# nogu-atsu/ENARF-GAN

Measured on AMD Instinct MI355X. Metric: rendered rays/sec (128^2, 64 samples/ray, 24 bones), higher is better.
Workload: dtype f32 (MLP products as 3-term split fp16 on MFMA, fp32 accumulate)

## Files before the change

enarf-gan_amd/csrc/enarf_tasks.h:

```cpp
#pragma once
#include "enarf_march.h"

namespace enarf {

constexpr unsigned ST_NONE = 0, ST_COARSE = 1, ST_FINE = 2;
__device__ __forceinline__ unsigned pack_ctl(unsigned gen, unsigned stage, unsigned tiles, unsigned next) {
    return (gen << 18) | (stage << 16) | (tiles << 8) | next;
}
__device__ __forceinline__ unsigned ctl_next(unsigned c) { return c & 0xFFu; }
__device__ __forceinline__ unsigned ctl_tiles(unsigned c) { return (c >> 8) & 0xFFu; }
__device__ __forceinline__ unsigned ctl_stage(unsigned c) { return (c >> 16) & 3u; }
__device__ __forceinline__ unsigned ctl_gen(unsigned c) { return c >> 18; }

constexpr int SH_QCUR = 0;
constexpr int SH_DEAD = 1;
constexpr int SH_INFLIGHT = 2;
constexpr int SH_PENDING = 3;
constexpr int SH_CTXB = 4;
constexpr int SH_SWITCHING = 5;
constexpr int SH_ERROR = 6;
constexpr int SH_FIRST = 7;
constexpr int SH_QCOUNTS = 8;
constexpr int SH_BTAB = SH_QCOUNTS + kQueues * kClasses;
constexpr int SH_PENDFLAG = SH_BTAB + 132;
constexpr int kSharedWords = SH_PENDFLAG + 16;
constexpr int kMaxSlots = 16;
constexpr unsigned kIdleLimit = 1u << 21;

template <int MODE>
__host__ __device__ inline int tasks_lds_floats(int P, int slots) {
    return lds_mlp_floats<MODE>() + 144 + P * kLdsPartStride + P * kLdsCanonStride + slots * kSlotWords + kSharedWords;
}

__device__ __forceinline__ unsigned wave_lds_add(unsigned *p, unsigned v, int lane) {
    unsigned r = 0;
    if (lane == 0) r = atomicAdd(p, v);
    return (unsigned)__builtin_amdgcn_readfirstlane((int)r);
}
__device__ __forceinline__ unsigned wave_lds_cas(unsigned *p, unsigned expect, unsigned desired, int lane) {
    unsigned r = 0;
    if (lane == 0) r = atomicCAS(p, expect, desired);
    return (unsigned)__builtin_amdgcn_readfirstlane((int)r);
}
__device__ __forceinline__ void lds_release() { __builtin_amdgcn_fence(__ATOMIC_RELEASE, "workgroup", "local"); }
__device__ __forceinline__ void lds_acquire() { __builtin_amdgcn_fence(__ATOMIC_ACQUIRE, "workgroup", "local"); }

struct TaskQueue {
    unsigned int *heads;
    const uint32_t *lists;
    const RayRec *recs;
    unsigned *sh;
    long long band;
    int home;
    __device__ __forceinline__ void init(void *workspace, int epoch, int B, int n, unsigned *shared, int tid) {
        unsigned int *wsh = reinterpret_cast<unsigned int *>(reinterpret_cast<char *>(workspace) + ws_header_off(epoch));
        heads = wsh + kWsHeadsOff;
        recs = reinterpret_cast<const RayRec *>(reinterpret_cast<const char *>(workspace) + ws_records_off());
        lists = reinterpret_cast<const uint32_t *>(reinterpret_cast<const char *>(workspace) + ws_list_off((long long)B * n));
        sh = shared;
        band = ws_band_size(B, n);
        home = xcc_id() & (kQueues - 1);
        if (tid < kQueues * kClasses) sh[SH_QCOUNTS + tid] = wsh[kWsCountsOff + tid];
    }
    __device__ __forceinline__ int pop(RayRec &rec, int lane) {
        int rid = -1;
        if (lane == 0) {
            unsigned cur = sh[SH_QCUR];
            int cls = (int)(cur >> 4), tries = (int)(cur & 15u);
            int lid = -1, idx = 0;
            while (cls < kClasses) {
                while (tries < kQueues) {
                    const int q = (home + tries) & (kQueues - 1);
                    const int l = q * kClasses + cls;
                    const unsigned len = sh[SH_QCOUNTS + l];
                    if (len != 0) {
                        const unsigned j = atomicAdd(heads + l * kWsHeadStride, 1u);
                        if (j < len) { lid = l; idx = (int)j; break; }
                    }
                    tries += 1;
                }
                if (lid >= 0) break;
                cls += 1;
                tries = 0;
            }
            atomicMax(&sh[SH_QCUR], (unsigned)(cls * 16 + tries));
            if (lid >= 0) rid = (int)lists[(size_t)lid * (size_t)band + (size_t)idx];
        }
        rid = __builtin_amdgcn_readfirstlane(rid);
        if (rid >= 0) rec = recs[rid];
        return rid;
    }
};

}

namespace enarf {

typedef const __attribute__((address_space(4))) enarf_render_args *RenderArgsK;
__device__ __forceinline__ RenderArgsK kernel_render_args() {
    return (RenderArgsK)__builtin_amdgcn_kernarg_segment_ptr();
}
__device__ __forceinline__ const enarf_render_args &render_args_ref(RenderArgsK a) { return *(const enarf_render_args *)a; }

struct MarchCtx {
    unsigned *slots;
    unsigned *sh;
    const float *btab;
    int nslots, nct, nft;
};

struct MarchCounters { unsigned pairs, tiles, rays, rounds, skipped; };

template <int SPL>
__device__ __forceinline__ void draw_sorted_uniforms(const enarf_render_args &a, uint32_t rid, int Nf, int lane, float usort[SPL]) {
    float esum[SPL];
    uint32_t r1_first = 0;
#pragma unroll
    for (int s = 0; s < SPL; ++s) {
        uint32_t rnd[4];
        philox4x32((uint32_t)(a.ray_id_base + rid), (uint32_t)((a.ray_id_base + rid) >> 32), (uint32_t)(64 * s + lane), 0x454E4152u, (uint32_t)a.seed, (uint32_t)(a.seed >> 32), rnd);
        esum[s] = (64 * s + lane < Nf) ? -__logf(1.0f - u32_to_unit(rnd[0])) : 0.0f;
        if (s == 0) r1_first = rnd[1];
    }
    wv_scan_incl<SPL>(esum, lane);
    const float etot = __shfl(esum[SPL - 1], 63) - __logf(1.0f - u32_to_unit((uint32_t)__shfl((int)r1_first, 0)));
#pragma unroll
    for (int s = 0; s < SPL; ++s) usort[s] = fminf(esum[s] / etot, 0.99999994f);
}

template <int SPL>
__device__ __forceinline__ void bins_from_cdf(int Nc, int Nf, const float cdf[SPL], const float usort[SPL], int lane, float bin[SPL]) {
    const float total = wv_get<SPL>(cdf, Nc - 1);
#pragma unroll
    for (int s = 0; s < SPL; ++s) {
        const float target = usort[s] * total;
        int lo = 0, hi = Nc - 1;
#pragma unroll
        for (int it = 0; it < 5 + SPL; ++it) {
            const int mid = (lo + hi) >> 1;
            const float c = wv_get<SPL>(cdf, mid);
            if (lo < hi) { if (c > target) hi = mid; else lo = mid + 1; }
        }
        const float c_hi = wv_get<SPL>(cdf, lo), c_lo = wv_get<SPL>(cdf, max(lo - 1, 0));
        const float below = (lo > 0) ? c_lo : 0.0f;
        const float frac = fminf(fmaxf((target - below) / (c_hi - below), 0.0f), 0.99999994f);
        bin[s] = (64 * s + lane < Nf) ? ((float)lo + frac) / (float)Nc : 3.0e38f;
    }
}

template <int SPL>
__device__ __forceinline__ void ray_sample_stage(const enarf_render_args &a, const float *l_btab, unsigned *sw, uint32_t rid,
                                                 float dmin, float dmax, const float usort[SPL], int mult_w, int lane) {
    const int P = a.P, Nc = a.Nc, Nf = a.Nf, n = a.n;
    const int b = (int)(rid / (uint32_t)n), ray = (int)(rid - (uint32_t)b * (uint32_t)n);
    const float *l_ch = reinterpret_cast<const float *>(sw + SL_CH), *l_cwmax = reinterpret_cast<const float *>(sw + SL_CWMAX);
    const uint32_t *l_cbits = sw + SL_CBITS;
    float *l_bins = reinterpret_cast<float *>(sw + SL_BINS);
    int *l_skip = reinterpret_cast<int *>(sw + SL_SKIP);
    float bin[SPL];
    float dd[SPL], cs[SPL], T[SPL], wgt[SPL], ws[SPL], wl[SPL], wr[SPL];
#pragma unroll
    for (int s = 0; s < SPL; ++s) {
        const int e = 64 * s + lane;
        const bool active = e < Nc;
        const int ci = min(e, Nc - 1);
        const float den = active ? density_head(l_ch[ci], l_cbits[ci], l_cwmax[ci], mult_w, P) : 0.0f;
        if (a.dbg_coarse_density && active) a.dbg_coarse_density[((size_t)b * n + ray) * Nc + e] = den;
        const float b0 = l_btab[ci], b1 = l_btab[ci + 1];
        const float delta = exact_lerp(dmin, dmax, b1) - exact_lerp(dmin, dmax, b0);
        dd[s] = active ? den * delta * a.render_scale : 0.0f;
        cs[s] = dd[s];
    }
    wv_scan_incl<SPL>(cs, lane);
#pragma unroll
    for (int s = 0; s < SPL; ++s) {
        T[s] = expf(-(cs[s] - dd[s]));
        wgt[s] = (64 * s + lane < Nc) ? T[s] * (1.0f - expf(-dd[s])) : 0.0f;
    }
    wv_prev<SPL>(wgt, wl, lane);
    wv_next<SPL>(wgt, wr, lane);
#pragma unroll
    for (int s = 0; s < SPL; ++s) {
        const int e = 64 * s + lane;
        if (e >= Nc - 1) wr[s] = 0.0f;
        ws[s] = (e < Nc) ? (fmaxf(wl[s], wgt[s]) + fmaxf(wgt[s], wr[s])) / 2.0f + 0.01f : 0.0f;
    }
    if (a.bins) {
#pragma unroll
        for (int s = 0; s < SPL; ++s) bin[s] = a.bins[((size_t)b * n + ray) * Nf + min(64 * s + lane, Nf - 1)];
    } else {
        float cdf[SPL];
#pragma unroll
        for (int s = 0; s < SPL; ++s) cdf[s] = ws[s];
        wv_scan_incl<SPL>(cdf, lane);
        bins_from_cdf<SPL>(Nc, Nf, cdf, usort, lane, bin);
    }
#pragma unroll
    for (int s = 0; s < SPL; ++s) {
        l_bins[64 * s + lane] = bin[s];
        if (a.dbg_bins && 64 * s + lane < Nf) a.dbg_bins[((size_t)b * n + ray) * Nf + 64 * s + lane] = bin[s];
    }
#pragma unroll
    for (int t = 0; t < 4 * SPL; ++t) {
        bool skip = false;
        if (a.early_stop_eps > 0.0f) {
            const float b_first = wv_get<SPL>(bin, min(16 * t, Nf - 1));
            const int jbin = min(max((int)(b_first * (float)Nc), 0), Nc - 1);
            skip = wv_get<SPL>(T, jbin) < a.early_stop_eps;
        }
        if (lane == 0) l_skip[t] = skip ? 1 : 0;
    }
}

template <int SPL>
__device__ __noinline__ void slot_sample_stage(RenderArgsK ak, const float *l_btab, unsigned *sw, int mult_w, int lane) {
    const enarf_render_args &a = render_args_ref(ak);
    const RayRec rec = *reinterpret_cast<const RayRec *>(sw + SL_REC);
    const uint32_t rid = sw[SL_RID];
    float usort[SPL] = {};
    if (!a.bins) draw_sorted_uniforms<SPL>(a, rid, a.Nf, lane, usort);
    ray_sample_stage<SPL>(a, l_btab, sw, rid, rec.dmin, rec.dmax, usort, mult_w, lane);
}

template <int SPL>
__device__ __forceinline__ void ray_composite_stage(const enarf_render_args &a, const unsigned *sw, uint32_t rid, float dmin,
                                                    float dmax, int mult_w, int lane) {
    const int P = a.P, Nf = a.Nf, n = a.n;
    const int b = (int)(rid / (uint32_t)n), ray = (int)(rid - (uint32_t)b * (uint32_t)n);
    const float *l_fh = reinterpret_cast<const float *>(sw + SL_FH), *l_fwmax = reinterpret_cast<const float *>(sw + SL_FWMAX);
    const float *l_bins = reinterpret_cast<const float *>(sw + SL_BINS);
    const uint32_t *l_fbits = sw + SL_FBITS;
    const bool dbgq = (a.dbg_fine_density != nullptr);
    float fdepth[SPL], dnext[SPL], den[SPL], cr[SPL], cg[SPL], cb[SPL], dd[SPL], cs[SPL];
#pragma unroll
    for (int s = 0; s < SPL; ++s) {
        const int e = 64 * s + lane;
        const int ci = min(e, Nf - 1);
        const bool have = e < (dbgq ? Nf : Nf - 1);
        const uint32_t bits = l_fbits[ci];
        den[s] = have ? density_head(l_fh[3 * kMaxSamples + ci], bits, l_fwmax[ci], mult_w, P) : 0.0f;
        cr[s] = tanhf(l_fh[ci]); cg[s] = tanhf(l_fh[kMaxSamples + ci]); cb[s] = tanhf(l_fh[2 * kMaxSamples + ci]);
        fdepth[s] = exact_lerp(dmin, dmax, l_bins[64 * s + lane]);
        if (dbgq && e < Nf) {
            const size_t o = ((size_t)b * n + ray) * Nf + e;
            a.dbg_fine_density[o] = den[s];
            if (a.dbg_fine_valid) a.dbg_fine_valid[o] = bits;
            if (a.dbg_fine_color) {
                a.dbg_fine_color[(((size_t)b * 3 + 0) * n + ray) * Nf + e] = cr[s];
                a.dbg_fine_color[(((size_t)b * 3 + 1) * n + ray) * Nf + e] = cg[s];
                a.dbg_fine_color[(((size_t)b * 3 + 2) * n + ray) * Nf + e] = cb[s];
            }
        }
    }
    wv_next<SPL>(fdepth, dnext, lane);
#pragma unroll
    for (int s = 0; s < SPL; ++s) {
        dd[s] = (64 * s + lane < Nf - 1) ? den[s] * (dnext[s] - fdepth[s]) * a.render_scale : 0.0f;
        cs[s] = dd[s];
    }
    wv_scan_incl<SPL>(cs, lane);
    float wgt[SPL], vr[SPL], vg[SPL], vb[SPL], vd[SPL];
#pragma unroll
    for (int s = 0; s < SPL; ++s) {
        const bool seg = 64 * s + lane < Nf - 1;
        const float T = expf(-(cs[s] - dd[s]));
        wgt[s] = seg ? T * (1.0f - expf(-dd[s])) : 0.0f;
        vr[s] = wgt[s] * cr[s]; vg[s] = wgt[s] * cg[s]; vb[s] = wgt[s] * cb[s];
        vd[s] = seg ? (wgt[s] * 1.0f) / fdepth[s] : 0.0f;
    }
    const float o_r = wv_sum<SPL>(vr), o_g = wv_sum<SPL>(vg), o_b = wv_sum<SPL>(vb);
    const float o_m = wv_sum<SPL>(wgt), o_d = wv_sum<SPL>(vd);
    if (lane == 0) {
        a.color[((size_t)b * 3 + 0) * n + ray] = o_r;
        a.color[((size_t)b * 3 + 1) * n + ray] = o_g;
        a.color[((size_t)b * 3 + 2) * n + ray] = o_b;
        a.mask[(size_t)b * n + ray] = o_m;
        a.disparity[(size_t)b * n + ray] = o_d;
    }
#pragma unroll
    for (int s = 0; s < SPL; ++s) {
        const int e = 64 * s + lane;
        if (a.fine_weights && e < Nf - 1) a.fine_weights[((size_t)b * n + ray) * (Nf - 1) + e] = wgt[s];
        if (a.fine_depth && e < Nf) a.fine_depth[((size_t)b * n + ray) * Nf + e] = fdepth[s];
    }
}

template <int SPL>
__device__ __noinline__ void slot_composite_stage(RenderArgsK ak, unsigned *sw, int mult_w, int lane) {
    const RayRec rec = *reinterpret_cast<const RayRec *>(sw + SL_REC);
    ray_composite_stage<SPL>(render_args_ref(ak), sw, sw[SL_RID], rec.dmin, rec.dmax, mult_w, lane);
}

struct RaySeg { float sx, sy, sz, ex, ey, ez; };
__device__ __forceinline__ RaySeg ray_segment(const RayRec &rec) {
    return {exact_mul(rec.dmin, rec.dx), exact_mul(rec.dmin, rec.dy), exact_mul(rec.dmin, rec.dz),
            exact_mul(rec.dmax, rec.dx), exact_mul(rec.dmax, rec.dy), exact_mul(rec.dmax, rec.dz)};
}

template <int MODE>
__device__ __forceinline__ void ray_tile(const enarf_render_args &a, const QueryCtx &S, const float *l_btab, const int *l_cand,
                                         int ncand, unsigned *sw, const RaySeg &g, bool fine, int t, int lane, MarchCounters &C) {
    const int Nc = a.Nc, Nf = a.Nf;
    const int j4 = lane >> 2, base = 16 * t, i = base + j4;
    const int N = fine ? Nf : Nc;
    const bool dbgq = (a.dbg_fine_density != nullptr);
    bool skip = false, active;
    float px, py, pz;
    if (!fine) {
        active = i < Nc;
        const int ci = min(i, Nc - 1);
        const float b0 = l_btab[ci], b1 = l_btab[ci + 1];
        px = exact_mid(exact_lerp(g.sx, g.ex, b1), exact_lerp(g.sx, g.ex, b0));
        py = exact_mid(exact_lerp(g.sy, g.ey, b1), exact_lerp(g.sy, g.ey, b0));
        pz = exact_mid(exact_lerp(g.sz, g.ez, b1), exact_lerp(g.sz, g.ez, b0));
    } else {
        skip = reinterpret_cast<const int *>(sw + SL_SKIP)[t] != 0;
        active = (i < (dbgq ? Nf : Nf - 1)) && !skip;
        const float bi = reinterpret_cast<const float *>(sw + SL_BINS)[min(i, Nf - 1)];
        px = exact_lerp(g.sx, g.ex, bi); py = exact_lerp(g.sy, g.ey, bi); pz = exact_lerp(g.sz, g.ez, bi);
    }
    const QueryDbg nodbg{nullptr, nullptr, 0, 0};
    f32x4 o;
    bool ran;
    uint32_t bits;
    float wmax;
    query_tile<MODE, false>(S, l_cand, ncand, px, py, pz, active, lane, o, ran, bits, wmax, nodbg, C.pairs, C.tiles, &C.rounds);
    float *heads = reinterpret_cast<float *>(sw + (fine ? SL_FH : SL_CH));
    if (lane < 16 && base + lane < N) {
        const int io = base + lane;
        if (fine) { heads[io] = o[0]; heads[kMaxSamples + io] = o[1]; heads[2 * kMaxSamples + io] = o[2]; heads[3 * kMaxSamples + io] = o[3]; }
        else heads[io] = o[3];
    }
    if (i < N && (lane & 3) == 0) {
        sw[(fine ? SL_FBITS : SL_CBITS) + i] = active ? bits : 0u;
        reinterpret_cast<float *>(sw + (fine ? SL_FWMAX : SL_CWMAX))[i] = wmax;
    }
    if (skip) C.skipped += 1;
}

template <int MODE>
__device__ __forceinline__ void ray_tile_task(const enarf_render_args &a, const MarchCtx &M, QueryCtx &S, unsigned *sw, bool fine,
                                              int t, int lane, MarchCounters &C) {
    const RayRec rec = *reinterpret_cast<const RayRec *>(sw + SL_REC);
    const uint32_t rid = (uint32_t)__builtin_amdgcn_readfirstlane((int)sw[SL_RID]);
    const int b = (int)(rid / (uint32_t)a.n);
    S.feat = a.feat_cl + (size_t)b * a.feat_batch_stride;
    S.mask = a.mask_planes + (size_t)b * a.mask_batch_stride;
    ray_tile<MODE>(a, S, M.btab, reinterpret_cast<const int *>(sw + SL_CAND), (int)sw[SL_NCAND], sw, ray_segment(rec), fine, t,
                   lane, C);
}

template <int SPL>
__device__ __forceinline__ void missed_ray_short_cut(RenderArgsK a, uint32_t rid, const RayRec &rec, const float cdf[SPL], int lane) {
    const int Nc = a->Nc, Nf = a->Nf, n = a->n;
    const int b = (int)(rid / (uint32_t)n), ray = (int)(rid - (uint32_t)b * (uint32_t)n);
    float bin[SPL];
    if (a->bins) {
#pragma unroll
        for (int s = 0; s < SPL; ++s) bin[s] = a->bins[((size_t)b * n + ray) * Nf + min(64 * s + lane, Nf - 1)];
    } else {
        float usort[SPL];
        draw_sorted_uniforms<SPL>(render_args_ref(a), rid, Nf, lane, usort);
        bins_from_cdf<SPL>(Nc, Nf, cdf, usort, lane, bin);
    }
    if (lane < 3) a->color[((size_t)b * 3 + lane) * n + ray] = 0.0f;
    if (lane == 3) a->mask[(size_t)b * n + ray] = 0.0f;
    if (lane == 4) a->disparity[(size_t)b * n + ray] = 0.0f;
#pragma unroll
    for (int s = 0; s < SPL; ++s) {
        const int e = 64 * s + lane;
        if (a->dbg_bins && e < Nf) a->dbg_bins[((size_t)b * n + ray) * Nf + e] = bin[s];
        if (a->fine_weights && e < Nf - 1) a->fine_weights[((size_t)b * n + ray) * (Nf - 1) + e] = 0.0f;
        if (a->fine_depth && e < Nf) a->fine_depth[((size_t)b * n + ray) * Nf + e] = exact_lerp(rec.dmin, rec.dmax, bin[s]);
    }
}

constexpr int kMissedChunk = 32;
template <int SPL>
__device__ __forceinline__ unsigned march_missed_rays(RenderArgsK ak, const float *l_btab, unsigned *scratch, int mult_w, int lane) {
    const int B = ak->B, n = ak->n, Nc = ak->Nc;
    const char *ws = reinterpret_cast<const char *>(ak->workspace);
    unsigned int *wsh = reinterpret_cast<unsigned int *>(const_cast<char *>(ws) + ws_header_off(ak->ws_epoch));
    const uint32_t *lists = reinterpret_cast<const uint32_t *>(ws + ws_list_off((long long)B * n));
    const RayRec *recs = reinterpret_cast<const RayRec *>(ws + ws_records_off());
    if (wsh[2] == 0u) return 0u;
    const long long band = ws_band_size(B, n);
    const int home = xcc_id() & (kQueues - 1);
    const bool general = ak->dbg_fine_density || ak->dbg_coarse_density;
    float cdf[SPL];
#pragma unroll
    for (int s = 0; s < SPL; ++s) cdf[s] = (64 * s + lane < Nc) ? (0.0f + 0.0f) / 2.0f + 0.01f : 0.0f;
    wv_scan_incl<SPL>(cdf, lane);
    unsigned done = 0;
    bool zeroed = false;
    for (int t = 0; t < kQueues; ++t) {
        const int l = ws_missed_list((home + t) & (kQueues - 1));
        const unsigned len = wsh[kWsCountsOff + l];
        if (len == 0u) continue;
        while (true) {
            unsigned j0 = 0;
            if (lane == 0) j0 = atomicAdd(wsh + kWsHeadsOff + l * kWsHeadStride, (unsigned)kMissedChunk);
            j0 = (unsigned)__builtin_amdgcn_readfirstlane((int)j0);
            if (j0 >= len) break;
            const unsigned j1 = min(j0 + (unsigned)kMissedChunk, len);
            for (unsigned j = j0; j < j1; ++j) {
                const uint32_t rid = (uint32_t)__builtin_amdgcn_readfirstlane((int)lists[(size_t)l * (size_t)band + j]);
                if (general) {
                    if (!zeroed) {
                        for (int i = lane; i < kSlotWords; i += 64) scratch[i] = 0u;
                        zeroed = true;
                    }
                    if (lane == 0) {
                        scratch[SL_RID] = rid;
                        *reinterpret_cast<RayRec *>(scratch + SL_REC) = recs[rid];
                    }
                    slot_sample_stage<SPL>(ak, l_btab, scratch, mult_w, lane);
                    slot_composite_stage<SPL>(ak, scratch, mult_w, lane);
                } else {
                    missed_ray_short_cut<SPL>(ak, rid, recs[rid], cdf, lane);
                }
                done += 1;
            }
        }
    }
    return done;
}

struct ImageCtx {
    const enarf_render_args *a;
    float *lds;
};

template <int MODE>
__device__ __forceinline__ void stage_image(RenderArgsK a, float *lds, int b, int lane) {
    QueryCtx tmp;
    float *unused;
    stage_common<MODE>(lds, tmp, unused, reinterpret_cast<const char *>(a->mlp_pack) + (size_t)b * kPackBytes,
                       a->parts + (size_t)b * a->P * kPartStride, a->canonical_pose, a->P, lane, 64);
}

__device__ __forceinline__ void publish_ray(const MarchCtx &M, unsigned *sw, int lane) {
    const RayRec rec = *reinterpret_cast<const RayRec *>(sw + SL_REC);
    const int ncand = build_cand_list(reinterpret_cast<int *>(sw + SL_CAND), rec.cand, lane);
    if (lane == 0) { sw[SL_NCAND] = (unsigned)ncand; sw[SL_DONE] = 0u; }
    lds_release();
    if (lane == 0) {
        const unsigned gen = (ctl_gen(sw[SL_CTL]) + 1u) & 0x3FFFu;
        __hip_atomic_store(&sw[SL_CTL], pack_ctl(gen, ST_COARSE, (unsigned)M.nct, 0u), __ATOMIC_RELAXED, __HIP_MEMORY_SCOPE_WORKGROUP);
    }
}

template <int MODE>
__device__ __forceinline__ void drain_point(RenderArgsK a, const MarchCtx &M, float *lds, int lane) {
    volatile unsigned *vsh = M.sh;
    while (true) {
        if (vsh[SH_PENDING] == 0u) return;
        if (wave_lds_cas(&M.sh[SH_SWITCHING], 0u, 1u, lane) != 0u) return;
        lds_acquire();
        unsigned best = 0xFFFFFFFFu;
        for (int s = 0; s < M.nslots; ++s)
            if (vsh[SH_PENDFLAG + s]) best = min(best, (unsigned)M.slots[s * kSlotWords + SL_RID]);
        if (best != 0xFFFFFFFFu) {
            const int b = (int)(best / (uint32_t)a->n);
            if ((unsigned)b != vsh[SH_CTXB]) {
                stage_image<MODE>(a, lds, b, lane);
                if (lane == 0) M.sh[SH_CTXB] = (unsigned)b;
            }
            lds_release();
            for (int s = 0; s < M.nslots; ++s) {
                unsigned *sw = M.slots + s * kSlotWords;
                if (vsh[SH_PENDFLAG + s] && (int)(sw[SL_RID] / (uint32_t)a->n) == b) {
                    if (lane == 0) { M.sh[SH_PENDFLAG + s] = 0u; atomicAdd(&M.sh[SH_PENDING], 0xFFFFFFFFu); atomicAdd(&M.sh[SH_INFLIGHT], 1u); }
                    publish_ray(M, sw, lane);
                }
            }
        }
        lds_release();
        if (lane == 0) __hip_atomic_store(&M.sh[SH_SWITCHING], 0u, __ATOMIC_RELAXED, __HIP_MEMORY_SCOPE_WORKGROUP);
        lds_release();
        lds_acquire();
        if (!(vsh[SH_INFLIGHT] == 0u && vsh[SH_PENDING] != 0u)) return;
    }
}

template <int MODE>
__device__ __forceinline__ void release_token(RenderArgsK a, const MarchCtx &M, float *lds, int lane) {
    lds_release();
    const unsigned before = wave_lds_add(&M.sh[SH_INFLIGHT], 0xFFFFFFFFu, lane);
    if (before == 1u) drain_point<MODE>(a, M, lds, lane);
}

template <int MODE>
__device__ __noinline__ unsigned refill_slot(RenderArgsK a, const MarchCtx M, TaskQueue tq, float *lds, int s, int lane) {
    unsigned popped = 0u;
    unsigned *sw = M.slots + s * kSlotWords;
    RayRec rec;
    int rid;
    volatile unsigned *vst = sw + SL_NEXT_STATE;
    unsigned ahead = *vst;
    while (ahead == 3u && reinterpret_cast<volatile unsigned *>(M.sh)[SH_ERROR] == 0u) { __builtin_amdgcn_s_sleep(2); ahead = *vst; }
    if (ahead == 3u) ahead = 2u;
    if (ahead == 1u) {
        lds_acquire();
        rid = (int)sw[SL_NEXT_RID];
        rec = *reinterpret_cast<const RayRec *>(sw + SL_NEXT_REC);
        lds_release();
        if (lane == 0) __hip_atomic_store(sw + SL_NEXT_STATE, 0u, __ATOMIC_RELAXED, __HIP_MEMORY_SCOPE_WORKGROUP);
    } else if (ahead == 2u) {
        rid = -1;
    } else {
        rid = tq.pop(rec, lane);
        if (rid >= 0) popped = 1u;
    }
    if (rid < 0) {
        if (lane == 0) atomicAdd(&M.sh[SH_DEAD], 1u);
        release_token<MODE>(a, M, lds, lane);
        return popped;
    }
    if (lane == 0) { sw[SL_RID] = (unsigned)rid; *reinterpret_cast<RayRec *>(sw + SL_REC) = rec; }
    const unsigned b = (unsigned)rid / (uint32_t)a->n;
    volatile unsigned *vsh = M.sh;
    if (b == vsh[SH_CTXB]) {
        publish_ray(M, sw, lane);
    } else {
        if (lane == 0) { M.sh[SH_PENDFLAG + s] = 1u; atomicAdd(&M.sh[SH_PENDING], 1u); }
        release_token<MODE>(a, M, lds, lane);
    }
    return popped;
}

__device__ __noinline__ unsigned prefetch_next_ray(TaskQueue tq, unsigned *sw, int lane) {
    if (wave_lds_cas(sw + SL_NEXT_STATE, 0u, 3u, lane) != 0u) return 0u;
    RayRec rec;
    const int rid = tq.pop(rec, lane);
    if (lane == 0 && rid >= 0) { sw[SL_NEXT_RID] = (unsigned)rid; *reinterpret_cast<RayRec *>(sw + SL_NEXT_REC) = rec; }
    lds_release();
    if (lane == 0) __hip_atomic_store(sw + SL_NEXT_STATE, rid >= 0 ? 1u : 2u, __ATOMIC_RELAXED, __HIP_MEMORY_SCOPE_WORKGROUP);
    return rid >= 0 ? 1u : 0u;
}

template <int MODE, int SPL, int NW>
__global__ __launch_bounds__(NW * 64, NW / 4) void march_kernel(const enarf_render_args a, int nslots, unsigned int *status) {
    extern __shared__ __attribute__((aligned(16))) float lds[];
    const int tid = threadIdx.x, lane = tid & 63, wave = tid >> 6;
    const int P = a.P, Nc = a.Nc, Nf = a.Nf;
    QueryCtx S;
    float *after;
    {
        float *l_mlp = lds, *l_bias = l_mlp + lds_mlp_floats<MODE>(), *l_parts = l_bias + 144;
        float *l_canon = l_parts + P * kLdsPartStride;
        after = l_canon + P * kLdsCanonStride;
        S.mlp = l_mlp; S.mlp_h = reinterpret_cast<const short *>(l_mlp); S.bias = l_bias; S.parts = l_parts; S.canon = l_canon;
    }
    S.feat = a.feat_cl; S.mask = a.mask_planes;
    S.H = a.H; S.W = a.W; S.P = P; S.mult_w = a.multiply_density_with_weight ? (a.uniform_part_weight ? 2 : 1) : 0;
    S.clamp_mask = a.clamp_mask; S.uniform_w = a.uniform_part_weight ? 1.0f / (float)P : 0.0f;
    MarchCtx M;
    M.slots = reinterpret_cast<unsigned *>(after);
    M.sh = M.slots + nslots * kSlotWords;
    M.btab = reinterpret_cast<const float *>(M.sh + SH_BTAB);
    M.nslots = nslots; M.nct = (Nc + 15) / 16; M.nft = (Nf + 15) / 16;
    TaskQueue tq;
    tq.init(a.workspace, a.ws_epoch, a.B, a.n, M.sh, tid);
    if (tid == 0) {
        M.sh[SH_QCUR] = 0u; M.sh[SH_DEAD] = 0u; M.sh[SH_PENDING] = 0u; M.sh[SH_CTXB] = 0xFFFFFFFFu; M.sh[SH_SWITCHING] = 0u;
        M.sh[SH_ERROR] = 0u;
        M.sh[SH_INFLIGHT] = (unsigned)nslots;
    }
    if (tid <= Nc) reinterpret_cast<float *>(M.sh + SH_BTAB)[tid] = linspace_sym(0.0f, 1.0f, Nc + 1, tid);
    for (int s = tid; s < nslots; s += NW * 64) {
        M.slots[s * kSlotWords + SL_CTL] = pack_ctl(0u, ST_NONE, 0u, 0u);
        M.slots[s * kSlotWords + SL_DONE] = 0u;
        M.slots[s * kSlotWords + SL_NEXT_STATE] = 0u;
        M.sh[SH_PENDFLAG + s] = 0u;
    }
    __syncthreads();

    MarchCounters C{0u, 0u, 0u, 0u, 0u};
    const RenderArgsK ak = kernel_render_args();
    if (wave < lds_mlp_floats<MODE>() / kSlotWords)
        C.rays += march_missed_rays<SPL>(ak, M.btab, reinterpret_cast<unsigned *>(lds) + wave * kSlotWords, S.mult_w, lane);
    __syncthreads();
    if (wave == 0) {
        RayRec rec;
        const int rid = tq.pop(rec, lane);
        if (lane == 0) {
            M.sh[SH_FIRST] = (unsigned)rid;
            if (rid >= 0) { M.slots[SL_RID] = (unsigned)rid; *reinterpret_cast<RayRec *>(M.slots + SL_REC) = rec; }
        }
        if (rid >= 0) C.rays += 1;
    }
    __syncthreads();
    const int first = (int)M.sh[SH_FIRST];
    if (first < 0) {
        if (a.counters && lane == 0 && C.rays) atomicAdd(&a.counters[2], (unsigned long long)C.rays);
        return;
    }
    {
        const int b0 = (int)((unsigned)first / (uint32_t)a.n);
        QueryCtx tmp;
        float *unused;
        stage_common<MODE>(lds, tmp, unused, reinterpret_cast<const char *>(a.mlp_pack) + (size_t)b0 * kPackBytes,
                           a.parts + (size_t)b0 * P * kPartStride, a.canonical_pose, P, tid, NW * 64);
        if (tid == 0) M.sh[SH_CTXB] = (unsigned)b0;
    }
    __syncthreads();
    if (wave == 0) publish_ray(M, M.slots, lane);
    for (int s = wave; s < nslots; s += NW)
        if (s != 0) C.rays += refill_slot<MODE>(ak, M, tq, lds, s, lane);

    volatile unsigned *vsl = M.slots;
    volatile unsigned *vsh = M.sh;
    unsigned idle = 0u;
    for (;;) {
        const unsigned c = (lane < nslots) ? vsl[lane * kSlotWords + SL_CTL] : 0u;
        const bool can = ctl_next(c) < ctl_tiles(c);
        const uint64_t bf = __ballot(can && ctl_stage(c) == ST_FINE), bc = __ballot(can && ctl_stage(c) == ST_COARSE);
        const uint64_t set = bf ? bf : bc;
        if (set) {
            const int start = wave % nslots;
            const uint64_t hi = (set >> start) << start;
            const int s = hi ? __builtin_ctzll(hi) : __builtin_ctzll(set);
            const unsigned old = (unsigned)__builtin_amdgcn_readlane((int)c, s);
            unsigned *sw = M.slots + s * kSlotWords;
            if (wave_lds_cas(&sw[SL_CTL], old, old + 1u, lane) != old) continue;
            lds_acquire();
            const bool fine = ctl_stage(old) == ST_FINE;
            idle = 0u;
            ray_tile_task<MODE>(a, M, S, sw, fine, (int)ctl_next(old), lane, C);
            lds_release();
            const unsigned d = wave_lds_add(&sw[SL_DONE], 1u, lane);
            if (d + 1u == ctl_tiles(old)) {
                lds_acquire();
                if (!fine) {
                    __builtin_amdgcn_s_setprio(3);
                    slot_sample_stage<SPL>(ak, M.btab, sw, S.mult_w, lane);
                    __builtin_amdgcn_s_setprio(0);
                    if (lane == 0) sw[SL_DONE] = 0u;
                    lds_release();
                    if (lane == 0)
                        __hip_atomic_store(&sw[SL_CTL], pack_ctl(ctl_gen(old), ST_FINE, (unsigned)M.nft, 0u), __ATOMIC_RELAXED,
                                           __HIP_MEMORY_SCOPE_WORKGROUP);
                    __builtin_amdgcn_s_setprio(1);
                    C.rays += prefetch_next_ray(tq, sw, lane);
                    __builtin_amdgcn_s_setprio(0);
                } else {
                    __builtin_amdgcn_s_setprio(3);
                    slot_composite_stage<SPL>(ak, sw, S.mult_w, lane);
                    C.rays += refill_slot<MODE>(ak, M, tq, lds, s, lane);
                    __builtin_amdgcn_s_setprio(0);
                }
            }
            continue;
        }
        if (vsh[SH_DEAD] >= (unsigned)nslots || vsh[SH_ERROR] != 0u) break;
        if (++idle > kIdleLimit) {
            if (lane == 0) {
                M.sh[SH_ERROR] = 1u;
                if (status) __hip_atomic_fetch_or(status, ENARF_STATUS_MARCH_WATCHDOG, __ATOMIC_RELAXED, __HIP_MEMORY_SCOPE_SYSTEM);
                if (a.counters) atomicAdd(&a.counters[7], 1ull);
                reinterpret_cast<unsigned int *>(reinterpret_cast<char *>(a.workspace) + ws_header_off(a.ws_epoch))[0] = 0xDEADu;
            }
            break;
        }
        __builtin_amdgcn_s_sleep(4);
    }
    if (a.counters && lane == 0) {
        atomicAdd(&a.counters[0], (unsigned long long)C.pairs);
        atomicAdd(&a.counters[1], (unsigned long long)C.tiles);
        atomicAdd(&a.counters[2], (unsigned long long)C.rays);
        atomicAdd(&a.counters[3], (unsigned long long)C.rounds);
        atomicAdd(&a.counters[4], (unsigned long long)C.skipped);
    }
}

}
```

Before: 66.97 million.

## Replace slot-scan tile scheduler with LDS ring queues of tile tokens

Waves used to poll every slot's control word and claim tiles by CAS on the per-slot counter. Now publishing a stage pushes one token per tile into a fine or a coarse ring buffer in LDS, and waves pop tokens by CAS on the ring head, with generation tags to drop stale tokens. Idle waves back off with an escalating sleep instead of a fixed one. This is meant to cut polling and CAS contention on slot words, but it adds ring bookkeeping and LDS space and carries ordering risk.

```diff
diff --git a/enarf-gan_amd/csrc/enarf_ring.h b/enarf-gan_amd/csrc/enarf_ring.h
--- /dev/null
+++ b/enarf-gan_amd/csrc/enarf_ring.h
@@ -0,0 +1,38 @@
+#pragma once
+
+#if defined(__HIPCC__) || defined(__CUDACC__)
+#define ENARF_RING_FN __host__ __device__ inline
+#else
+#define ENARF_RING_FN inline
+#endif
+
+namespace enarf {
+
+constexpr int kMaxSlots = 16;
+constexpr int kRingMaxTiles = 8;
+constexpr int kRingLog2 = 7;
+constexpr int kRingSize = 1 << kRingLog2;
+static_assert(kRingSize == kMaxSlots * kRingMaxTiles, "a ring holds every slot's largest stage");
+
+constexpr int RQ_HEAD_FINE = 0, RQ_TAIL_FINE = 1, RQ_HEAD_COARSE = 2, RQ_TAIL_COARSE = 3;
+constexpr int RQ_FINE = 4, RQ_COARSE = RQ_FINE + kRingSize;
+constexpr int kRingWords = RQ_COARSE + kRingSize;
+constexpr unsigned kRingEmptyEntry = 0xFFFF0000u;
+
+ENARF_RING_FN unsigned ring_index(unsigned pos) { return pos & (unsigned)(kRingSize - 1); }
+ENARF_RING_FN unsigned ring_lap(unsigned pos) { return (pos >> kRingLog2) & 0xFFFFu; }
+ENARF_RING_FN unsigned ring_token(unsigned pos, unsigned gen, unsigned slot, unsigned tile) {
+    return (ring_lap(pos) << 16) | ((gen & 0xFFu) << 8) | ((slot & 15u) << 4) | (tile & 15u);
+}
+ENARF_RING_FN unsigned token_tile(unsigned t) { return t & 15u; }
+ENARF_RING_FN unsigned token_slot(unsigned t) { return (t >> 4) & 15u; }
+ENARF_RING_FN unsigned token_gen(unsigned t) { return (t >> 8) & 0xFFu; }
+ENARF_RING_FN bool ring_entry_ready(unsigned entry, unsigned pos) { return (entry >> 16) == ring_lap(pos); }
+ENARF_RING_FN bool token_is_current(unsigned t, unsigned gen) { return token_gen(t) == (gen & 0xFFu); }
+ENARF_RING_FN int ring_pick(unsigned head_fine, unsigned tail_fine, unsigned head_coarse, unsigned tail_coarse) {
+    if (head_fine != tail_fine) return 0;
+    if (head_coarse != tail_coarse) return 1;
+    return -1;
+}
+
+}
diff --git a/enarf-gan_amd/csrc/enarf_tasks.h b/enarf-gan_amd/csrc/enarf_tasks.h
--- a/enarf-gan_amd/csrc/enarf_tasks.h
+++ b/enarf-gan_amd/csrc/enarf_tasks.h
@@ -1,5 +1,6 @@
 #pragma once
 #include "enarf_march.h"
+#include "enarf_ring.h"
 
 namespace enarf {
 
@@ -23,13 +24,13 @@
 constexpr int SH_QCOUNTS = 8;
 constexpr int SH_BTAB = SH_QCOUNTS + kQueues * kClasses;
 constexpr int SH_PENDFLAG = SH_BTAB + 132;
-constexpr int kSharedWords = SH_PENDFLAG + 16;
-constexpr int kMaxSlots = 16;
+constexpr int kSharedWords = SH_PENDFLAG + kMaxSlots;
 constexpr unsigned kIdleLimit = 1u << 21;
 
 template <int MODE>
 __host__ __device__ inline int tasks_lds_floats(int P, int slots) {
-    return lds_mlp_floats<MODE>() + 144 + P * kLdsPartStride + P * kLdsCanonStride + slots * kSlotWords + kSharedWords;
+    return lds_mlp_floats<MODE>() + 144 + P * kLdsPartStride + P * kLdsCanonStride + slots * kSlotWords + kSharedWords +
+           kRingWords + 3;
 }
 
 __device__ __forceinline__ unsigned wave_lds_add(unsigned *p, unsigned v, int lane) {
@@ -44,6 +45,24 @@
 }
 __device__ __forceinline__ void lds_release() { __builtin_amdgcn_fence(__ATOMIC_RELEASE, "workgroup", "local"); }
 __device__ __forceinline__ void lds_acquire() { __builtin_amdgcn_fence(__ATOMIC_ACQUIRE, "workgroup", "local"); }
+
+__device__ __forceinline__ void ring_push(unsigned *rq, bool fine, unsigned slot, unsigned gen, int ntiles, int lane) {
+    lds_release();
+    const unsigned t0 = wave_lds_add(&rq[fine ? RQ_TAIL_FINE : RQ_TAIL_COARSE], (unsigned)ntiles, lane);
+    if (lane < ntiles) {
+        const unsigned pos = t0 + (unsigned)lane;
+        __hip_atomic_store(&rq[(fine ? RQ_FINE : RQ_COARSE) + ring_index(pos)], ring_token(pos, gen, slot, (unsigned)lane),
+                           __ATOMIC_RELAXED, __HIP_MEMORY_SCOPE_WORKGROUP);
+    }
+}
+__device__ __forceinline__ bool ring_take(unsigned *rq, bool fine, unsigned head, unsigned &token, int lane) {
+    const unsigned e = (unsigned)__builtin_amdgcn_readfirstlane(
+        (int)reinterpret_cast<volatile unsigned *>(rq)[(fine ? RQ_FINE : RQ_COARSE) + ring_index(head)]);
+    if (!ring_entry_ready(e, head)) return false;
+    if (wave_lds_cas(&rq[fine ? RQ_HEAD_FINE : RQ_HEAD_COARSE], head, head + 1u, lane) != head) return false;
+    token = e;
+    return true;
+}
 
 struct TaskQueue {
     unsigned int *heads;
@@ -105,6 +124,7 @@
 struct MarchCtx {
     unsigned *slots;
     unsigned *sh;
+    unsigned *rq;
     const float *btab;
     int nslots, nct, nft;
 };
@@ -439,15 +459,13 @@
                        a->parts + (size_t)b * a->P * kPartStride, a->canonical_pose, a->P, lane, 64);
 }
 
-__device__ __forceinline__ void publish_ray(const MarchCtx &M, unsigned *sw, int lane) {
+__device__ __forceinline__ void publish_ray(const MarchCtx &M, int s, int lane) {
+    unsigned *sw = M.slots + s * kSlotWords;
     const RayRec rec = *reinterpret_cast<const RayRec *>(sw + SL_REC);
     const int ncand = build_cand_list(reinterpret_cast<int *>(sw + SL_CAND), rec.cand, lane);
-    if (lane == 0) { sw[SL_NCAND] = (unsigned)ncand; sw[SL_DONE] = 0u; }
-    lds_release();
-    if (lane == 0) {
-        const unsigned gen = (ctl_gen(sw[SL_CTL]) + 1u) & 0x3FFFu;
-        __hip_atomic_store(&sw[SL_CTL], pack_ctl(gen, ST_COARSE, (unsigned)M.nct, 0u), __ATOMIC_RELAXED, __HIP_MEMORY_SCOPE_WORKGROUP);
-    }
+    const unsigned gen = (ctl_gen(reinterpret_cast<volatile unsigned *>(sw)[SL_CTL]) + 1u) & 0x3FFFu;
+    if (lane == 0) { sw[SL_NCAND] = (unsigned)ncand; sw[SL_DONE] = 0u; sw[SL_CTL] = pack_ctl(gen, ST_COARSE, (unsigned)M.nct, 0u); }
+    ring_push(M.rq, false, (unsigned)s, gen, M.nct, lane);
 }
 
 template <int MODE>
@@ -471,7 +489,7 @@
                 unsigned *sw = M.slots + s * kSlotWords;
                 if (vsh[SH_PENDFLAG + s] && (int)(sw[SL_RID] / (uint32_t)a->n) == b) {
                     if (lane == 0) { M.sh[SH_PENDFLAG + s] = 0u; atomicAdd(&M.sh[SH_PENDING], 0xFFFFFFFFu); atomicAdd(&M.sh[SH_INFLIGHT], 1u); }
-                    publish_ray(M, sw, lane);
+                    publish_ray(M, s, lane);
                 }
             }
         }
@@ -521,7 +539,7 @@
     const unsigned b = (unsigned)rid / (uint32_t)a->n;
     volatile unsigned *vsh = M.sh;
     if (b == vsh[SH_CTXB]) {
-        publish_ray(M, sw, lane);
+        publish_ray(M, s, lane);
     } else {
         if (lane == 0) { M.sh[SH_PENDFLAG + s] = 1u; atomicAdd(&M.sh[SH_PENDING], 1u); }
         release_token<MODE>(a, M, lds, lane);
@@ -558,6 +576,7 @@
     MarchCtx M;
     M.slots = reinterpret_cast<unsigned *>(after);
     M.sh = M.slots + nslots * kSlotWords;
+    M.rq = reinterpret_cast<unsigned *>(lds) + ((M.sh + kSharedWords - reinterpret_cast<unsigned *>(lds) + 3) & ~3);
     M.btab = reinterpret_cast<const float *>(M.sh + SH_BTAB);
     M.nslots = nslots; M.nct = (Nc + 15) / 16; M.nft = (Nf + 15) / 16;
     TaskQueue tq;
@@ -574,6 +593,7 @@
         M.slots[s * kSlotWords + SL_NEXT_STATE] = 0u;
         M.sh[SH_PENDFLAG + s] = 0u;
     }
+    for (int i = tid; i < kRingWords; i += NW * 64) M.rq[i] = (i < RQ_FINE) ? 0u : kRingEmptyEntry;
     __syncthreads();
 
     MarchCounters C{0u, 0u, 0u, 0u, 0u};
@@ -605,42 +625,42 @@
         if (tid == 0) M.sh[SH_CTXB] = (unsigned)b0;
     }
     __syncthreads();
-    if (wave == 0) publish_ray(M, M.slots, lane);
+    if (wave == 0) publish_ray(M, 0, lane);
     for (int s = wave; s < nslots; s += NW)
         if (s != 0) C.rays += refill_slot<MODE>(ak, M, tq, lds, s, lane);
 
-    volatile unsigned *vsl = M.slots;
+    typedef unsigned u32x4 __attribute__((ext_vector_type(4)));
     volatile unsigned *vsh = M.sh;
-    unsigned idle = 0u;
+    unsigned idle = 0u, naps = 0u;
     for (;;) {
-        const unsigned c = (lane < nslots) ? vsl[lane * kSlotWords + SL_CTL] : 0u;
-        const bool can = ctl_next(c) < ctl_tiles(c);
-        const uint64_t bf = __ballot(can && ctl_stage(c) == ST_FINE), bc = __ballot(can && ctl_stage(c) == ST_COARSE);
-        const uint64_t set = bf ? bf : bc;
-        if (set) {
-            const int start = wave % nslots;
-            const uint64_t hi = (set >> start) << start;
-            const int s = hi ? __builtin_ctzll(hi) : __builtin_ctzll(set);
-            const unsigned old = (unsigned)__builtin_amdgcn_readlane((int)c, s);
+        const u32x4 q = *reinterpret_cast<volatile u32x4 *>(M.rq);
+        const unsigned hf = (unsigned)__builtin_amdgcn_readfirstlane((int)q[RQ_HEAD_FINE]);
+        const unsigned tf = (unsigned)__builtin_amdgcn_readfirstlane((int)q[RQ_TAIL_FINE]);
+        const unsigned hc = (unsigned)__builtin_amdgcn_readfirstlane((int)q[RQ_HEAD_COARSE]);
+        const unsigned tc = (unsigned)__builtin_amdgcn_readfirstlane((int)q[RQ_TAIL_COARSE]);
+        const int pick = ring_pick(hf, tf, hc, tc);
+        unsigned token = 0u;
+        bool fine = pick == 0;
+        bool got = fine && ring_take(M.rq, true, hf, token, lane);
+        if (!got && hc != tc) { fine = false; got = ring_take(M.rq, false, hc, token, lane); }
+        if (got) {
+            lds_acquire();
+            const int s = (int)token_slot(token);
             unsigned *sw = M.slots + s * kSlotWords;
-            if (wave_lds_cas(&sw[SL_CTL], old, old + 1u, lane) != old) continue;
-            lds_acquire();
-            const bool fine = ctl_stage(old) == ST_FINE;
-            idle = 0u;
-            ray_tile_task<MODE>(a, M, S, sw, fine, (int)ctl_next(old), lane, C);
+            const unsigned gen = ctl_gen((unsigned)__builtin_amdgcn_readfirstlane((int)reinterpret_cast<volatile unsigned *>(sw)[SL_CTL]));
+            if (!token_is_current(token, gen)) continue;
+            idle = 0u; naps = 0u;
+            ray_tile_task<MODE>(a, M, S, sw, fine, (int)token_tile(token), lane, C);
             lds_release();
             const unsigned d = wave_lds_add(&sw[SL_DONE], 1u, lane);
-            if (d + 1u == ctl_tiles(old)) {
+            if (d + 1u == (unsigned)(fine ? M.nft : M.nct)) {
                 lds_acquire();
                 if (!fine) {
                     __builtin_amdgcn_s_setprio(3);
                     slot_sample_stage<SPL>(ak, M.btab, sw, S.mult_w, lane);
                     __builtin_amdgcn_s_setprio(0);
-                    if (lane == 0) sw[SL_DONE] = 0u;
-                    lds_release();
-                    if (lane == 0)
-                        __hip_atomic_store(&sw[SL_CTL], pack_ctl(ctl_gen(old), ST_FINE, (unsigned)M.nft, 0u), __ATOMIC_RELAXED,
-                                           __HIP_MEMORY_SCOPE_WORKGROUP);
+                    if (lane == 0) { sw[SL_DONE] = 0u; sw[SL_CTL] = pack_ctl(gen, ST_FINE, (unsigned)M.nft, 0u); }
+                    ring_push(M.rq, true, (unsigned)s, gen, M.nft, lane);
                     __builtin_amdgcn_s_setprio(1);
                     C.rays += prefetch_next_ray(tq, sw, lane);
                     __builtin_amdgcn_s_setprio(0);
@@ -663,7 +683,12 @@
             }
             break;
         }
-        __builtin_amdgcn_s_sleep(4);
+        if (pick >= 0) continue;
+        if (naps == 0u) __builtin_amdgcn_s_sleep(1);
+        else if (naps == 1u) __builtin_amdgcn_s_sleep(2);
+        else if (naps == 2u) __builtin_amdgcn_s_sleep(4);
+        else __builtin_amdgcn_s_sleep(8);
+        naps += 1u;
     }
     if (a.counters && lane == 0) {
         atomicAdd(&a.counters[0], (unsigned long long)C.pairs);
```

After: 67.06 million, median of 2. About the same (+0.1%).
